# junejunejune/c_orb_slam

Measured on AMD Instinct MI355X. Metric: tracking FPS + ORB matches/sec, KITTI-00 stereo; local-BA iter/sec, higher is better.
Workload: dtype u8

## Files before the change

c_orb_slam_amd/csrc/octree.hip:

```cpp
#include "octree.hpp"

#include <cstdlib>

namespace orbgpu {

constexpr int OCT_TMAX = 1024;
constexpr int kOctCellsMax = kOctKMax / 2;

struct OctShared {
    int16_t x0[2 * kOctNMax], y0[2 * kOctNMax], x1[2 * kOctNMax], y1[2 * kOctNMax];
    uint16_t cnt[2 * kOctNMax], seq[2 * kOctNMax], kbeg[2 * kOctNMax];
    int16_t prv[2 * kOctNMax], nxt[2 * kOctNMax];
    int ia[4 * kOctNMax];
    uint16_t vpos[4 * kOctNMax];
    uint16_t er[kOctNMax], eidx[kOctNMax];
    uint16_t vs[kOctNMax], vs2[kOctNMax];
    uint32_t sk[kOctNMax];
    uint16_t knode[kOctKMax], arena[kOctKMax];
    alignas(16) uint16_t tmp[kOctKMax];
    int wsum[OCT_TMAX / 64];
    int head, size, nfree, m, newm, seqctr, flag;
};

template <int T, class Flag, class Put>
__device__ __forceinline__ int oct_scan(int n, Flag flag, Put put, int* wsum) {
    const int t = threadIdx.x, lane = t & 63, wid = t >> 6;
    const int per = (n + T - 1) / T;
    const int a = min(n, t * per), e = min(n, a + per);
    int local = 0;
    for (int i = a; i < e; i++) local += flag(i) ? 1 : 0;
    int incl = local;
#pragma unroll
    for (int o = 1; o < 64; o <<= 1) {
        const int y = __shfl_up(incl, o, 64);
        if (lane >= o) incl += y;
    }
    if (lane == 63) wsum[wid] = incl;
    __syncthreads();
    int off = 0, total = 0;
#pragma unroll
    for (int w = 0; w < T / 64; w++) {
        const int s = wsum[w];
        if (w < wid) off += s;
        total += s;
    }
    int ex = off + incl - local;
    for (int i = a; i < e; i++)
        if (flag(i)) put(i, ex++);
    __syncthreads();
    return total;
}

template <int T, class Val, class Put>
__device__ __forceinline__ int oct_scan_val(int n, Val val, Put put, int* wsum) {
    const int t = threadIdx.x, lane = t & 63, wid = t >> 6;
    const int per = (n + T - 1) / T;
    const int a = min(n, t * per), e = min(n, a + per);
    int local = 0;
    for (int i = a; i < e; i++) local += val(i);
    int incl = local;
#pragma unroll
    for (int o = 1; o < 64; o <<= 1) {
        const int y = __shfl_up(incl, o, 64);
        if (lane >= o) incl += y;
    }
    if (lane == 63) wsum[wid] = incl;
    __syncthreads();
    int off = 0, total = 0;
#pragma unroll
    for (int w = 0; w < T / 64; w++) {
        const int s = wsum[w];
        if (w < wid) off += s;
        total += s;
    }
    int ex = off + incl - local;
    for (int i = a; i < e; i++) {
        put(i, ex);
        ex += val(i);
    }
    __syncthreads();
    return total;
}

__device__ __forceinline__ void oct_child_rect(const OctShared& S, int p, int q, int& a0, int& b0, int& a1, int& b1) {
    const int X0 = S.x0[p], Y0 = S.y0[p], X1 = S.x1[p], Y1 = S.y1[p];
    const int halfX = (int)ceilf((float)(X1 - X0) / 2), halfY = (int)ceilf((float)(Y1 - Y0) / 2);
    const int mx = X0 + halfX, my = Y0 + halfY;
    a0 = (q & 1) ? mx : X0;
    a1 = (q & 1) ? X1 : mx;
    b0 = (q & 2) ? my : Y0;
    b1 = (q & 2) ? Y1 : my;
}

__device__ __forceinline__ int oct_quadrant(const OctShared& S, int p, uint32_t pk) {
    const int halfX = (int)ceilf((float)(S.x1[p] - S.x0[p]) / 2), halfY = (int)ceilf((float)(S.y1[p] - S.y0[p]) / 2);
    const int mx = S.x0[p] + halfX, my = S.y0[p] + halfY;
    const int x = (int)(pk & 0xfff), y = (int)((pk >> 12) & 0xfff);
    return (x < mx) ? (y < my ? 0 : 2) : (y < my ? 1 : 3);
}

__device__ __forceinline__ int oct_best_key(uint32_t pk, int k) { return (int)((pk >> 24) << 16) | (0xffff - k); }

template <int T>
__global__ void __launch_bounds__(T) k_octree(OctInput in, int nlevels, const OctLevelDev* __restrict__ lv,
                                                 uint32_t* __restrict__ jobsel, int* __restrict__ jobcnt, int jcap,
                                                 uint16_t* __restrict__ gscratch, size_t gstride, int* __restrict__ err) {
    __shared__ OctShared S;
    ORBGPU_PROF_START;
#ifdef ORBGPU_PROF
    struct JobTimer {
        unsigned long long t0;
        int lvl;
        __device__ ~JobTimer() {
            if (threadIdx.x == 0) {
                const unsigned long long c = clock64() - t0;
                atomicMax(&g_orbgpu_prof[10], (c << 4) | (unsigned long long)lvl);
                atomicAdd(&g_orbgpu_prof[11], c);
                atomicAdd(&g_orbgpu_prof[12], 1ull);
            }
        }
    } jt{(unsigned long long)clock64(), (int)blockIdx.x / ((int)gridDim.x / nlevels)};
#endif
    const int B = (int)gridDim.x / nlevels;
    const int l = (int)blockIdx.x / B, b = (int)blockIdx.x - l * B, job = b * nlevels + l;
    const int tid = threadIdx.x;
    const int cb = in.lcb[l], nc = in.lcb[l + 1] - cb;
    const int* cnt = in.counts + (size_t)b * in.ncells + cb;
    if (nc + 1 > 4 * kOctNMax || nc > kOctCellsMax) {
        if (tid == 0) {
            jobcnt[job] = 0;
            atomicOr(err, 2);
        }
        return;
    }
    int* cdelta = reinterpret_cast<int*>(S.tmp);
    const int n = oct_scan_val<T>(
        nc, [&](int i) { return cnt[i]; },
        [&](int i, int o) {
            S.ia[i] = o;
            cdelta[i] = in.cell_slot[cb + i] - in.cell_slot[cb] - o;
        },
        S.wsum);
    const size_t base = (size_t)b * in.slots_per_image + (size_t)in.cell_slot[cb];
    if (n <= 0 || n > 0xffff) {
        if (tid == 0) {
            jobcnt[job] = 0;
            if (n > 0xffff) atomicOr(err, 2);
        }
        return;
    }
    {
        const uint32_t* sl = in.slots + base;
        uint32_t* dst = in.packed + base;
        constexpr int U = 4;
        for (int k0 = tid; k0 < n; k0 += U * T) {
            uint32_t v[U];
#pragma unroll
            for (int u = 0; u < U; u++) {
                const int k = k0 + u * T;
                if (k < n) {
                    int lo = 0, hi = nc - 1;
                    while (lo < hi) {
                        const int mid = (lo + hi + 1) >> 1;
                        if (S.ia[mid] <= k) lo = mid;
                        else hi = mid - 1;
                    }
                    v[u] = sl[k + cdelta[lo]];
                }
            }
#pragma unroll
            for (int u = 0; u < U; u++)
                if (k0 + u * T < n) dst[k0 + u * T] = v[u];
        }
        if (tid == 0) atomicAdd(in.g_total, n);
    }
    __syncthreads();
    const uint32_t* src = in.packed + base;
    const OctLevelDev L = lv[l];
    const int N = L.N;
    uint16_t* knode = S.knode;
    uint16_t* arena = S.arena;
    uint16_t* tmp = S.tmp;
    if (n > kOctKMax) {
        knode = gscratch + base;
        arena = knode + gstride;
        tmp = arena + gstride;
    }
    const int W = L.maxX - L.minX, Hh = L.maxY - L.minY;
    const int nIni = (int)roundf((float)W / (float)Hh);
    if (nIni < 1 || nIni > kOctNMax) {
        if (tid == 0) {
            jobcnt[job] = 0;
            atomicOr(err, 4);
        }
        return;
    }
    const float hX = (float)W / (float)nIni;
    for (int i = tid; i < nIni; i += T) S.ia[i] = 0;
    __syncthreads();
    for (int k = tid; k < n; k += T) {
        const uint32_t pk = src[k];
        int ib = (int)((float)(pk & 0xfff) / hX);
        ib = min(ib, nIni - 1);
        knode[k] = (uint16_t)ib;
        atomicAdd(&S.ia[ib], 1);
    }
    __syncthreads();
    int cur = 0;
    int Sz = oct_scan<T>(
        nIni, [&](int i) { return S.ia[i] > 0; },
        [&](int i, int r) {
            S.x0[r] = (int16_t)(int)(hX * (float)i);
            S.x1[r] = (int16_t)(int)(hX * (float)(i + 1));
            S.y0[r] = 0;
            S.y1[r] = (int16_t)Hh;
            S.cnt[r] = (uint16_t)S.ia[i];
            S.seq[r] = (uint16_t)i;
            S.er[i] = (uint16_t)r;
        },
        S.wsum);
    for (int k = tid; k < n; k += T) knode[k] = S.er[knode[k]];
    int seqbase = nIni;
    int phase2 = 0, m = 0;
    __syncthreads();
    ORBGPU_PROF_MARK(0);
    for (;;) {
        const int prevSize = Sz;
        const int nE = oct_scan<T>(
            Sz, [&](int i) { return S.cnt[cur + i] > 1; },
            [&](int i, int r) {
                S.er[i] = (uint16_t)r;
                S.eidx[r] = (uint16_t)i;
            },
            S.wsum);
        ORBGPU_PROF_COUNT(9);
        if (nE == 0) break;
        for (int v = tid; v < 4 * nE; v += T) S.ia[v] = 0;
        __syncthreads();
        for (int k = tid; k < n; k += T) {
            const int p = knode[k];
            if (S.cnt[cur + p] > 1) {
                const int v = 4 * S.er[p] + oct_quadrant(S, cur + p, src[k]);
                tmp[k] = (uint16_t)v;
                atomicAdd(&S.ia[v], 1);
            } else {
                tmp[k] = 0xffff;
            }
        }
        __syncthreads();
        const int nC = oct_scan<T>(
            4 * nE, [&](int v) { return S.ia[v] > 0; }, [&](int v, int r) { S.vpos[v] = (uint16_t)r; }, S.wsum);
        const int nb = kOctNMax - cur;
        const int nNM = oct_scan<T>(
            Sz, [&](int i) { return S.cnt[cur + i] == 1; }, [&](int i, int r) { S.er[i] = (uint16_t)(nC + r); },
            S.wsum);
        if (nC + nNM > kOctNMax) {
            if (tid == 0) {
                jobcnt[job] = 0;
                atomicOr(err, 8);
            }
            return;
        }
        for (int v = tid; v < 4 * nE; v += T) {
            const int c = S.ia[v];
            if (c > 0) {
                const int t = S.vpos[v], pos = nC - 1 - t, parent = cur + S.eidx[v >> 2];
                int a0, b0, a1, b1;
                oct_child_rect(S, parent, v & 3, a0, b0, a1, b1);
                S.x0[nb + pos] = (int16_t)a0;
                S.y0[nb + pos] = (int16_t)b0;
                S.x1[nb + pos] = (int16_t)a1;
                S.y1[nb + pos] = (int16_t)b1;
                S.cnt[nb + pos] = (uint16_t)c;
                S.seq[nb + pos] = (uint16_t)(seqbase + t);
                S.vpos[v] = (uint16_t)pos;
            }
        }
        for (int i = tid; i < Sz; i += T)
            if (S.cnt[cur + i] == 1) {
                const int pos = S.er[i];
                S.x0[nb + pos] = S.x0[cur + i];
                S.y0[nb + pos] = S.y0[cur + i];
                S.x1[nb + pos] = S.x1[cur + i];
                S.y1[nb + pos] = S.y1[cur + i];
                S.cnt[nb + pos] = 1;
                S.seq[nb + pos] = S.seq[cur + i];
            }
        __syncthreads();
        const int nToExpand = oct_scan<T>(
            4 * nE, [&](int v) { return S.ia[v] > 1; }, [&](int v, int r) { S.vs[r] = (uint16_t)S.vpos[v]; },
            S.wsum);
        for (int k = tid; k < n; k += T) {
            const int v = tmp[k];
            knode[k] = v != 0xffff ? S.vpos[v] : S.er[knode[k]];
        }
        seqbase += nC;
        cur = nb;
        Sz = nC + nNM;
        __syncthreads();
        if (Sz >= N || Sz == prevSize) break;
        if (Sz + nToExpand * 3 > N) {
            phase2 = 1;
            m = nToExpand;
            break;
        }
    }
    ORBGPU_PROF_MARK(1);
    if (phase2) {
        const int nb = kOctNMax - cur;
        {
            oct_scan_val<T>(
                Sz, [&](int i) { return (int)S.cnt[cur + i]; }, [&](int i, int ex) { S.kbeg[cur + i] = (uint16_t)ex; },
                S.wsum);
            for (int i = tid; i < Sz; i += T) {
                S.ia[i] = 0;
                S.prv[cur + i] = (int16_t)(i > 0 ? cur + i - 1 : -1);
                S.nxt[cur + i] = (int16_t)(i + 1 < Sz ? cur + i + 1 : -1);
            }
            if (tid == 0) {
                S.head = Sz > 0 ? cur : -1;
                S.size = Sz;
                S.nfree = nb;
                S.seqctr = seqbase;
                S.m = m;
                S.flag = 0;
            }
            for (int i = tid; i < m; i += T) S.vs[i] = (uint16_t)(cur + S.vs[i]);
            __syncthreads();
            for (int k = tid; k < n; k += T) {
                const int p = knode[k];
                arena[S.kbeg[cur + p] + atomicAdd(&S.ia[p], 1)] = (uint16_t)k;
            }
            __syncthreads();
        }
        ORBGPU_PROF_MARK(2);
        for (;;) {
            ORBGPU_PROF_COUNT(8);
            const int prevSize = S.size;
            const int mm = S.m;
            for (int i = tid; i < mm; i += T) {
                const int id = S.vs[i];
                S.sk[i] = ((uint32_t)S.cnt[id] << 16) | S.seq[id];
            }
            __syncthreads();
            for (int i = tid; i < mm; i += T) {
                const uint32_t ki = S.sk[i];
                int r = 0;
                for (int j = 0; j < mm; j++) r += S.sk[j] < ki ? 1 : 0;
                S.vs2[r] = S.vs[i];
            }
            for (int i = tid; i < 4 * mm; i += T) S.ia[i] = 0;
            if (tid == 0) S.newm = 0;
            __syncthreads();
            ORBGPU_PROF_MARK(3);
            const int tot = oct_scan_val<T>(
                mm, [&](int j) { return (int)S.cnt[S.vs2[j]]; }, [&](int j, int ex) { S.er[j] = (uint16_t)ex; },
                S.wsum);
            auto owner = [&](int t) {
                int lo = 0, hi = mm - 1;
                while (lo < hi) {
                    const int mid = (lo + hi + 1) >> 1;
                    if ((int)S.er[mid] <= t) lo = mid;
                    else hi = mid - 1;
                }
                return lo;
            };
            for (int t = tid; t < tot; t += T) {
                const int j = owner(t), p = S.vs2[j], pos = S.kbeg[p] + (t - S.er[j]);
                const int k = arena[pos];
                const int q = oct_quadrant(S, p, src[k]);
                tmp[t] = (uint16_t)k;
                knode[t] = (uint16_t)(4 * j + q);
                atomicAdd(&S.ia[4 * j + q], 1);
            }
            __syncthreads();
            for (int j = tid; j < mm; j += T) {
                int start = S.kbeg[S.vs2[j]];
#pragma unroll
                for (int q = 0; q < 4; q++) {
                    S.vpos[4 * j + q] = (uint16_t)start;
                    start += S.ia[4 * j + q];
                    S.ia[4 * j + q] = 0;
                }
            }
            __syncthreads();
            for (int t = tid; t < tot; t += T) {
                const int v = knode[t];
                arena[S.vpos[v] + atomicAdd(&S.ia[v], 1)] = tmp[t];
            }
            __syncthreads();
            ORBGPU_PROF_MARK(4);
            if (tid == 0) {
                int head = S.head, size = S.size, nfree = S.nfree, seqctr = S.seqctr, newm = 0, flag = 0;
                for (int j = mm - 1; j >= 0; j--) {
                    const int p = S.vs2[j];
                    int c4[4];
#pragma unroll
                    for (int q = 0; q < 4; q++) c4[q] = S.ia[4 * j + q];
                    for (int q = 0; q < 4; q++) {
                        const int c = c4[q];
                        if (c > 0) {
                            const int id = nfree++;
                            if (nfree > 2 * kOctNMax || id == cur) {
                                flag = 1;
                                break;
                            }
                            int a0, b0, a1, b1;
                            oct_child_rect(S, p, q, a0, b0, a1, b1);
                            S.x0[id] = (int16_t)a0;
                            S.y0[id] = (int16_t)b0;
                            S.x1[id] = (int16_t)a1;
                            S.y1[id] = (int16_t)b1;
                            S.cnt[id] = (uint16_t)c;
                            S.seq[id] = (uint16_t)(seqctr++);
                            S.kbeg[id] = S.vpos[4 * j + q];
                            S.prv[id] = -1;
                            S.nxt[id] = (int16_t)head;
                            if (head >= 0) S.prv[head] = (int16_t)id;
                            head = id;
                            size++;
                            if (c > 1) S.vs[newm++] = (uint16_t)id;
                        }
                    }
                    if (flag) break;
                    const int pp = S.prv[p], pn = S.nxt[p];
                    if (pp >= 0) S.nxt[pp] = (int16_t)pn;
                    else head = pn;
                    if (pn >= 0) S.prv[pn] = (int16_t)pp;
                    S.prv[p] = -2;
                    size--;
                    if (size >= N) break;
                }
                S.head = head;
                S.size = size;
                S.nfree = nfree;
                S.seqctr = seqctr;
                S.newm = newm;
                S.flag = flag;
            }
            __syncthreads();
            ORBGPU_PROF_MARK(5);
            if (S.flag) {
                if (tid == 0) {
                    jobcnt[job] = 0;
                    atomicOr(err, 8);
                }
                return;
            }
            if (S.size >= N || S.size == prevSize) break;
            if (tid == 0) S.m = S.newm;
            __syncthreads();
        }
        const int n2 = S.nfree - nb;
        const int sz = oct_scan<T>(
            n2 + Sz,
            [&](int u) {
                const int id = u < n2 ? nb + n2 - 1 - u : cur + (u - n2);
                return S.prv[id] != -2;
            },
            [&](int u, int r) { S.vpos[r] = (uint16_t)(u < n2 ? nb + n2 - 1 - u : cur + (u - n2)); }, S.wsum);
        if (sz > jcap) {
            if (tid == 0) {
                jobcnt[job] = 0;
                atomicOr(err, 16);
            }
            return;
        }
        for (int i = tid; i < sz; i += T) {
            const int id = S.vpos[i];
            const int kb = S.kbeg[id], kc = S.cnt[id];
            for (int t = 0; t < kc; t++) tmp[kb + t] = (uint16_t)i;
            S.ia[i] = -1;
        }
        __syncthreads();
        for (int pos = tid; pos < n; pos += T) {
            const int k = arena[pos];
            atomicMax(&S.ia[tmp[pos]], oct_best_key(src[k], k));
        }
        __syncthreads();
        for (int i = tid; i < sz; i += T) {
            const int k = 0xffff - (S.ia[i] & 0xffff);
            jobsel[(size_t)job * jcap + i] = src[k];
        }
        if (tid == 0) jobcnt[job] = sz;
        ORBGPU_PROF_MARK(6);
        return;
    }
    if (Sz > jcap) {
        if (tid == 0) {
            jobcnt[job] = 0;
            atomicOr(err, 16);
        }
        return;
    }
    for (int i = tid; i < Sz; i += T) S.ia[i] = -1;
    __syncthreads();
    for (int k = tid; k < n; k += T) atomicMax(&S.ia[knode[k]], oct_best_key(src[k], k));
    __syncthreads();
    for (int i = tid; i < Sz; i += T) {
        const int k = 0xffff - (S.ia[i] & 0xffff);
        jobsel[(size_t)job * jcap + i] = src[k];
    }
    if (tid == 0) jobcnt[job] = Sz;
    ORBGPU_PROF_MARK(7);
}

__global__ void __launch_bounds__(64) k_sel_build(const uint32_t* __restrict__ jobsel, const int* __restrict__ jobcnt,
                                                  int nlevels, int jcap, int cap, int2* __restrict__ sel, int selcap,
                                                  int* __restrict__ nout, int* __restrict__ err) {
    const int b = blockIdx.x, lane = threadIdx.x;
    const int c = lane < nlevels ? jobcnt[b * nlevels + lane] : 0;
    int incl = c;
#pragma unroll
    for (int o = 1; o < 64; o <<= 1) {
        const int y = __shfl_up(incl, o, 64);
        if (lane >= o) incl += y;
    }
    const int total = __shfl(incl, 63, 64);
    if (lane == 0) {
        nout[b] = total;
        if (total > cap || total > selcap) atomicOr(err, 1);
    }
    if (total > cap || total > selcap) return;
    for (int l = 0; l < nlevels; l++) {
        const int cl = __shfl(c, l, 64), off = __shfl(incl - c, l, 64);
        const uint32_t* js = jobsel + (size_t)(b * nlevels + l) * jcap;
        for (int i = lane; i < cl; i += 64)
            sel[(size_t)b * selcap + off + i] = make_int2((int)js[i], (b << 20) | (l << 16) | (off + i));
    }
}

int octree_prof_read(unsigned long long* out16) {
#ifdef ORBGPU_PROF
    unsigned long long v[32];
    ORB_HIP_CHECK(hipMemcpyFromSymbol(v, HIP_SYMBOL(g_orbgpu_prof), sizeof(v)));
    for (int i = 0; i < 16; i++) out16[i] = v[i];
    unsigned long long z[32] = {};
    ORB_HIP_CHECK(hipMemcpyToSymbol(HIP_SYMBOL(g_orbgpu_prof), z, sizeof(z)));
    return 0;
#else
    (void)out16;
    return -1;
#endif
}

int octree_launch(const OctInput& in, int B, int nlevels, const OctLevelDev* lv, uint32_t* jobsel, int* jobcnt, int jcap,
                  uint16_t* gscratch, size_t gstride, int cap, int2* sel, int selcap, int* nout, int* err,
                  hipStream_t s) {
    static const int nt = [] {
        const char* e = getenv("ORBGPU_OCT_T");
        const int v = e ? atoi(e) : 512;
        return v == 256 || v == 1024 ? v : 512;
    }();
    if (nt == 1024)
        hipLaunchKernelGGL(k_octree<1024>, dim3(B * nlevels), dim3(1024), 0, s, in, nlevels, lv, jobsel, jobcnt,
                           jcap, gscratch, gstride, err);
    else if (nt == 512)
        hipLaunchKernelGGL(k_octree<512>, dim3(B * nlevels), dim3(512), 0, s, in, nlevels, lv, jobsel, jobcnt,
                           jcap, gscratch, gstride, err);
    else
        hipLaunchKernelGGL(k_octree<256>, dim3(B * nlevels), dim3(256), 0, s, in, nlevels, lv, jobsel, jobcnt,
                           jcap, gscratch, gstride, err);
    hipLaunchKernelGGL(k_sel_build, dim3(B), dim3(64), 0, s, (const uint32_t*)jobsel, (const int*)jobcnt, nlevels,
                       jcap, cap, sel, selcap, nout, err);
    ORB_HIP_CHECK(hipGetLastError());
    return 0;
}

}
```

c_orb_slam_amd/csrc/octree.hpp:

```cpp
#pragma once
#include <hip/hip_runtime.h>

#include <cstdint>

#include "orb_common.hpp"

namespace orbgpu {

constexpr int kOctNMax = 640;
constexpr int kOctKMax = 4096;

struct OctLevelDev {
    int minX, maxX, minY, maxY, N;
};

int octree_prof_read(unsigned long long* out16);

struct OctInput {
    const uint32_t* slots;
    size_t slots_per_image;
    const int* counts;
    const int* cell_slot;
    const int* lcb;
    int ncells;
    uint32_t* packed;
    int* g_total;
};

int octree_launch(const OctInput& in, int B, int nlevels, const OctLevelDev* lv, uint32_t* jobsel, int* jobcnt, int jcap,
                  uint16_t* gscratch, size_t gstride, int cap, int2* sel, int selcap, int* nout, int* err,
                  hipStream_t s);

}
```

c_orb_slam_amd/csrc/orb_extract.hip:

```cpp
#include "orb_extract.hpp"

#include <algorithm>
#include <atomic>
#include <chrono>
#include <cmath>
#include <cstring>
#include <thread>

namespace orbgpu {

__constant__ int8_t c_pattern[256 * 4];
__constant__ int8_t c_disc[2 * 1024];
__constant__ int c_ndisc;
__constant__ int c_umax[16];
__constant__ int c_gauss[7];

static const int8_t kPattern[256 * 4] = {
#include "brief_pattern.inc"
};

__device__ __forceinline__ int xcd_tile(int bid, int nb) { return (bid & 7) * (nb >> 3) + (bid >> 3); }
static inline unsigned grid8(int n) { return (unsigned)((n + 7) & ~7); }
constexpr int kFastSplitLevel = 3;

// ... 1444 lines not shown
    ORB_HIP_CHECK(hipMalloc(&d_blur_, blur_bytes_ * B));
    ORB_HIP_CHECK(hipMemset(d_blur_, 0, blur_bytes_ * B));
    ORB_HIP_CHECK(hipMalloc(&d_slots_, slots_per_image_ * 4 * B));
    ORB_HIP_CHECK(hipMalloc(&d_counts_, cells_.size() * 4 * B));
    ORB_HIP_CHECK(hipMalloc(&d_cells_, cells_.size() * sizeof(CellDesc)));
    ORB_HIP_CHECK(hipMemcpy(d_cells_, cells_.data(), cells_.size() * sizeof(CellDesc), hipMemcpyHostToDevice));
    ORB_HIP_CHECK(hipMalloc(&d_groups_, groups_.size() * sizeof(CellGroup)));
    ORB_HIP_CHECK(hipMemcpy(d_groups_, groups_.data(), groups_.size() * sizeof(CellGroup), hipMemcpyHostToDevice));
    ORB_HIP_CHECK(hipMalloc(&d_tiles_, tiles_.size() * sizeof(BlurTile)));
    ORB_HIP_CHECK(hipMemcpy(d_tiles_, tiles_.data(), tiles_.size() * sizeof(BlurTile), hipMemcpyHostToDevice));
    {
        std::vector<int> cs(cells_.size());
        for (size_t c = 0; c < cells_.size(); c++) cs[c] = cells_[c].slot_off;
        ORB_HIP_CHECK(hipMalloc(&d_cellslot_, std::max<size_t>(cs.size(), 1) * 4));
        ORB_HIP_CHECK(hipMemcpy(d_cellslot_, cs.data(), cs.size() * 4, hipMemcpyHostToDevice));
    }
    ORB_HIP_CHECK(hipMalloc(&d_lcb_, level_cell_begin_.size() * 4));
    ORB_HIP_CHECK(hipMemcpy(d_lcb_, level_cell_begin_.data(), level_cell_begin_.size() * 4, hipMemcpyHostToDevice));
    if (slots_per_image_ * B > ((size_t)1 << 30)) return -1;
    packed_cap_ = (int)(slots_per_image_ * B);
    ORB_HIP_CHECK(hipMalloc(&d_packed_, (size_t)packed_cap_ * 4));
    ORB_HIP_CHECK(hipMalloc(&d_hdr_, (size_t)B * (nlevels_ + 2) * 4 + 64));
    d_gtotal_ = (int*)((char*)d_hdr_ + (size_t)B * (nlevels_ + 2) * 4);
    d_gtotal_alias_ = true;
    sel_cap_ = B * std::max(nfeatures_ * 2 + 64, 256);
    ORB_HIP_CHECK(hipMalloc(&d_sel_, (size_t)sel_cap_ * sizeof(int2)));
    std::vector<LevelDev> ld(nlevels_);
    for (int l = 0; l < nlevels_; l++) {
        ld[l].off = levels_[l].off;
        ld[l].pitch = levels_[l].pitch;
        ld[l].scale = scale_[l];
        ld[l].boff = levels_[l].boff;
        ld[l].bpitch = levels_[l].bpitch;
        ld[l].kp_size = (float)(int)(kPatch * scale_[l]);
    }
    if (nlevels_ > kMaxLevels) return -1;
    for (int l = 0; l < nlevels_; l++) levelArgs_.lv[l] = ld[l];
    ORB_HIP_CHECK(hipMalloc(&d_levels_, ld.size() * sizeof(LevelDev)));
    ORB_HIP_CHECK(hipMemcpy(d_levels_, ld.data(), ld.size() * sizeof(LevelDev), hipMemcpyHostToDevice));
    ORB_HIP_CHECK(hipMalloc(&d_tabs_, std::max<size_t>(tabs.size(), 16)));
    if (!tabs.empty()) ORB_HIP_CHECK(hipMemcpy(d_tabs_, tabs.data(), tabs.size(), hipMemcpyHostToDevice));
    F(d_jobsel_); F(d_jobcnt_); F(d_octlv_); F(d_gscr_); F(d_nout_);
    jcap_ = 0;
    std::vector<OctLevelDev> ol(nlevels_);
    for (int l = 0; l < nlevels_; l++) {
        ol[l].minX = kEdge - 3;
        ol[l].maxX = levels_[l].w - kEdge + 3;
        ol[l].minY = kEdge - 3;
        ol[l].maxY = levels_[l].h - kEdge + 3;
        ol[l].N = nPerLevel_[l];
        jcap_ = std::max(jcap_, nPerLevel_[l] + 8);
    }
    if (jcap_ > kOctNMax) return -1;
    selcap_ = jcap_ * nlevels_;
    ORB_HIP_CHECK(hipMalloc(&d_octlv_, ol.size() * sizeof(OctLevelDev)));
    ORB_HIP_CHECK(hipMemcpy(d_octlv_, ol.data(), ol.size() * sizeof(OctLevelDev), hipMemcpyHostToDevice));
    ORB_HIP_CHECK(hipMalloc(&d_jobsel_, (size_t)B * nlevels_ * jcap_ * 4));
    ORB_HIP_CHECK(hipMalloc(&d_jobcnt_, (size_t)B * nlevels_ * 4));
    ORB_HIP_CHECK(hipMalloc(&d_gscr_, (size_t)packed_cap_ * 3 * 2));
    ORB_HIP_CHECK(hipMalloc(&d_nout_, (size_t)(B + 1) * 4));
    ORB_HIP_CHECK(hipFree(d_sel_));
    d_sel_ = nullptr;
    sel_cap_ = selcap_ * B;
    ORB_HIP_CHECK(hipMalloc(&d_sel_, (size_t)sel_cap_ * sizeof(int2)));
    if (h_nout_) (void)hipHostFree(h_nout_);
    ORB_HIP_CHECK(hipHostMalloc((void**)&h_nout_, (size_t)(B + 1) * 4));
    geomW_ = W;
    geomH_ = H;
    return 0;
}

int Extractor::extract(const uint8_t* imgs, int B, int W, int H, int step, size_t img_stride,
                       bool imgs_on_device, orb_kp* kps, uint8_t* desc, int cap, bool out_on_device,
                       int* n_out, const uint8_t* const* list) {
    if (B <= 0 || B > maxB_ || W <= 0 || H <= 0) return -1;
    if (W > maxW_ || H > maxH_) return -1;
    if (int e = setup_geometry(W, H)) return e;
    hipStream_t s = stream_;
    const uint8_t* src = imgs;
    if (!imgs_on_device) {
        const size_t need = img_stride * (B - 1) + (size_t)step * (H - 1) + W;
        if (need > in_cap_) {
            if (d_in_) (void)hipFree(d_in_);
            ORB_HIP_CHECK(hipMalloc(&d_in_, need));
            in_cap_ = need;
        }
        if (h_in_) ORB_HIP_CHECK(hipEventSynchronize(ev_[0]));
        if (need > h_in_cap_) {
            if (h_in_) (void)hipHostFree(h_in_);
            h_in_ = nullptr;
            h_in_cap_ = 0;
            ORB_HIP_CHECK(hipHostMalloc(&h_in_, need));
            h_in_cap_ = need;
        }
        if (list) {
            const size_t one = (size_t)step * (H - 1) + W;
            for (int b = 0; b < B; b++) std::memcpy((uint8_t*)h_in_ + img_stride * b, list[b], one);
        } else {
            std::memcpy(h_in_, imgs, need);
        }
        ORB_HIP_CHECK(hipMemcpyAsync(d_in_, h_in_, need, hipMemcpyHostToDevice, s));
        src = (const uint8_t*)d_in_;
    }
    ORB_HIP_CHECK(hipEventRecord(ev_[0], s));
    const int ncells = (int)cells_.size();
    if (work_B_ != B && build_work(B)) return -2;
    const bool split = fastSplit_ && work_part_[0] > 0 && work_part_[1] > 0;
    int planFlags = (split ? kPlanFastSplit : 0) | (evBlur_ ? kPlanBlurSide : 0) | (B >= 8 ? kPlanTile32 : 0);
    int planChainFrom = 0;
    {
        const LevelHost& L0 = levels_[0];
        const int n = (L0.pitch / 16) * L0.ph;
// ... 31 lines not shown
            const LevelHost& P = levels_[l - 1];
            const uint8_t* T = (const uint8_t*)d_tabs_;
            const int v = B >= 8 ? 1 : 0, pb = v * (nlevels_ + 1) + l;
            const int nt = ptile_n_[v * nlevels_ + l];
            auto kern = v ? k_pyr_resize<kPyrTileH[1]> : k_pyr_resize<kPyrTileH[0]>;
            hipLaunchKernelGGL(kern, dim3(grid8(nt), B), dim3(256), plds_[v * nlevels_ + l], s, (uint8_t*)d_pyr_, img_bytes_,
                               P.off, P.pitch, L.off, L.pitch, L.ph, L.w, L.h,
                               (const int*)(T + tab_off_[l][0]), (const short2*)(T + tab_off_[l][1]),
                               (const int2*)(T + tab_off_[l][2]), (const short2*)(T + tab_off_[l][3]),
                               (const PyrTile*)d_ptiles_ + ptile_begin_[pb], nt);
        }
        if (!flow && lend < nlevels_) {
            const uint8_t* T = (const uint8_t*)d_chain_;
            const LevelHost& P = levels_[lend - 1];
            hipLaunchKernelGGL(k_pyr_chain, dim3(chainK_, B), dim3(256), chainLds_, s, (uint8_t*)d_pyr_, img_bytes_,
                               (long long)P.off, P.pitch, P.w, (const ChainLevel*)T, nlevels_ - lend,
                               (const int4*)(T + chainStripOff_), (const uint16_t*)(T + chainRowOff_),
                               (const uint8_t*)d_tabs_, chainSrcLds_, chainSrcRp_);
        }
    }
    ORB_HIP_CHECK(hipGetLastError());
    ORB_HIP_CHECK(hipEventRecord(ev_[1], s));
    static const bool blurEarly = [] {
        const char* e = getenv("ORBGPU_BLUR_EARLY");
        return e && e[0] == '1';
    }();
    if (blurEarly && !evBlur_) {
        planFlags |= kPlanBlurEarly;
        hipLaunchKernelGGL(k_blur7, dim3(grid8((int)tiles_.size()), B), dim3(256), 0, s, (const uint8_t*)d_pyr_,
                           (uint8_t*)d_blur_, img_bytes_, blur_bytes_, (const BlurTile*)d_tiles_, (int)tiles_.size());
    }
    if (evBlur_) {
        ORB_HIP_CHECK(hipStreamWaitEvent(side_, ev_[1], 0));
        hipLaunchKernelGGL(k_blur7, dim3(grid8((int)tiles_.size()), B), dim3(256), 0, side_, (const uint8_t*)d_pyr_,
                           (uint8_t*)d_blur_, img_bytes_, blur_bytes_, (const BlurTile*)d_tiles_, (int)tiles_.size());
        ORB_HIP_CHECK(hipEventRecord(evBlur_, side_));
    }
    if (split) {
        hipLaunchKernelGGL(k_fast_cells, dim3(work_part_[1]), dim3(256), 0, s, (const uint8_t*)d_pyr_, img_bytes_,
                           (const CellGroup*)d_groups_, iniTh_, minTh_, (uint32_t*)d_slots_, slots_per_image_,
                           (int*)d_counts_, ncells, (const int*)d_work_ + work_part_[0]);
        ORB_HIP_CHECK(hipStreamWaitEvent(s, evFastA_, 0));
    } else {
        hipLaunchKernelGGL(k_fast_cells, dim3(work_n_), dim3(256), 0, s, (const uint8_t*)d_pyr_, img_bytes_,
                           (const CellGroup*)d_groups_, iniTh_, minTh_, (uint32_t*)d_slots_, slots_per_image_,
                           (int*)d_counts_, ncells, (const int*)d_work_);
    }
    ORB_HIP_CHECK(hipGetLastError());
    ORB_HIP_CHECK(hipEventRecord(ev_[3], s));
    ORB_HIP_CHECK(hipEventRecord(ev_[4], s));
    int* d_err = (int*)d_nout_ + B;
    OctInput oin{(const uint32_t*)d_slots_, slots_per_image_, (const int*)d_counts_, (const int*)d_cellslot_,
                 (const int*)d_lcb_, ncells, (uint32_t*)d_packed_, d_gtotal_};
    if (int e = octree_launch(oin, B, nlevels_, (const OctLevelDev*)d_octlv_, (uint32_t*)d_jobsel_, (int*)d_jobcnt_,
                              jcap_, (uint16_t*)d_gscr_, (size_t)packed_cap_, cap, (int2*)d_sel_, selcap_,
                              (int*)d_nout_, d_err, s))
        return e;
    ORB_HIP_CHECK(hipEventRecord(ev_[5], s));
    if (evBlur_)
        ORB_HIP_CHECK(hipStreamWaitEvent(s, evBlur_, 0));
    else if (!blurEarly)
        hipLaunchKernelGGL(k_blur7, dim3(grid8((int)tiles_.size()), B), dim3(256), 0, s, (const uint8_t*)d_pyr_,
                           (uint8_t*)d_blur_, img_bytes_, blur_bytes_, (const BlurTile*)d_tiles_, (int)tiles_.size());
    ORB_HIP_CHECK(hipEventRecord(ev_[2], s));
    orb_kp_dev* okps = (orb_kp_dev*)kps;
    uint8_t* odesc = desc;
    if (!out_on_device) {
        const size_t nk = (size_t)B * cap;
        if (nk > out_cap_) {
            if (d_kps_) (void)hipFree(d_kps_);
            if (d_desc_) (void)hipFree(d_desc_);
            ORB_HIP_CHECK(hipMalloc(&d_kps_, nk * sizeof(orb_kp_dev)));
            ORB_HIP_CHECK(hipMalloc(&d_desc_, nk * 32));
            out_cap_ = nk;
        }
        okps = (orb_kp_dev*)d_kps_;
        odesc = (uint8_t*)d_desc_;
    }
    {
        const int gx = (selcap_ + 3) / 4;
        const int nwg = B >= 8 ? gx * 8 * ((B + 7) / 8) : gx * B;
        hipLaunchKernelGGL(k_orient_desc, dim3(nwg), dim3(256), 0, s, (const uint8_t*)d_pyr_,
                           (const uint8_t*)d_blur_, img_bytes_, blur_bytes_, (const int2*)d_sel_, selcap_,
                           (const int*)d_nout_, levelArgs_, okps, odesc, cap, gx, B);
    }
    ORB_HIP_CHECK(hipGetLastError());
    ORB_HIP_CHECK(hipMemcpyAsync(h_nout_, d_nout_, (size_t)(B + 1) * 4, hipMemcpyDeviceToHost, s));
    ORB_HIP_CHECK(hipEventRecord(ev_[6], s));
    ORB_HIP_CHECK(stream_wait(s));
    const int err = h_nout_[B];
    for (int b = 0; b < B; b++) n_out[b] = h_nout_[b];
    if (err & 1) return -3;
    if (err) return -1;
    if (!out_on_device) {
        for (int b = 0; b < B; b++) {
            if (n_out[b] == 0) continue;
            ORB_HIP_CHECK(hipMemcpyAsync(kps + (size_t)b * cap, okps + (size_t)b * cap, (size_t)n_out[b] * sizeof(orb_kp_dev),
                                         hipMemcpyDeviceToHost, s));
            ORB_HIP_CHECK(hipMemcpyAsync(desc + (size_t)b * cap * 32, odesc + (size_t)b * cap * 32, (size_t)n_out[b] * 32,
                                         hipMemcpyDeviceToHost, s));
        }
        ORB_HIP_CHECK(stream_wait(s));
    }
    last_B_ = B;
    planFlags_ = planFlags;
    planChainFrom_ = planChainFrom;
    return 0;
}

// ... 66 lines not shown
```

c_orb_slam_amd/csrc/orb_extract.hpp:

```cpp
#pragma once
#include <atomic>
#include <condition_variable>
#include <cstddef>
#include <cstdint>
#include <mutex>
#include <thread>
#include <vector>
#include <array>

#include "orb_common.hpp"
#include "octree.hpp"
#include "../../include/orbslam_gpu.h"

namespace orbgpu {

struct orb_kp_dev {
    float x, y, size, angle, response;
    int32_t octave, class_id;
};
static_assert(sizeof(orb_kp_dev) == 28, "cv::KeyPoint layout");

struct CellDesc {
    int r0, r1, c0, c1;
    int offx, offy;
// ... 104 lines not shown
    int maxW_ = 0, maxH_ = 0, maxB_ = 0;
    int geomW_ = -1, geomH_ = -1;
    std::vector<LevelHost> levels_;
    LevelArgs levelArgs_{};
    std::vector<CellDesc> cells_;
    std::vector<CellGroup> groups_;
    std::vector<int> level_cell_begin_;
    std::vector<BlurTile> tiles_;
    std::vector<PyrTile> ptiles_;
    std::vector<int> ptile_begin_, ptile_n_, plds_;
    std::vector<int> ptile_th_;
    bool flow_ = false;
    int* d_flowcnt_ = nullptr;
    int flowBands_[2] = {0, 0}, flowLds_[2] = {0, 0};
    FlowArgs flow_args(int v, int B) const;
    int plan_chain(const std::vector<std::vector<int>>& yr);
    bool chain_ = false;
    int chainK_ = 0, chainLds_ = 0, chainFrom_ = 0, chainSrcLds_ = 0, chainSrcRp_ = 0;
    std::vector<std::vector<int>> xofsAll_;
    std::vector<std::vector<short>> xalAll_;
    size_t chainStripOff_ = 0, chainRowOff_ = 0;
    std::vector<uint8_t> chainTab_;
    void* d_chain_ = nullptr;
    void* d_cellslot_ = nullptr;
    std::vector<std::array<size_t, 4>> tab_off_;
    size_t img_bytes_ = 0, blur_bytes_ = 0, slots_per_image_ = 0;
    int packed_cap_ = 0, sel_cap_ = 0;
    int last_B_ = 0;
    int planFlags_ = 0, planChainFrom_ = 0;

    hipStream_t stream_ = nullptr;
    bool ownStream_ = true;
    int lent_ = 0;
    hipEvent_t ev_[7] = {};
    hipStream_t side_ = nullptr;
    hipEvent_t evBlur_ = nullptr;
    bool fastSplit_ = false;
    hipEvent_t evPyrA_ = nullptr, evFastA_ = nullptr;
    void *d_in_ = nullptr, *d_pyr_ = nullptr, *d_blur_ = nullptr, *d_slots_ = nullptr, *d_counts_ = nullptr;
    void *d_ptiles_ = nullptr;
    void *d_cells_ = nullptr, *d_tiles_ = nullptr, *d_lcb_ = nullptr, *d_packed_ = nullptr, *d_hdr_ = nullptr;
    void *d_sel_ = nullptr, *d_levels_ = nullptr, *d_tabs_ = nullptr, *d_kps_ = nullptr, *d_desc_ = nullptr;
    int* d_gtotal_ = nullptr;
    void* d_work_ = nullptr;
    void* d_groups_ = nullptr;
    int work_B_ = -1, work_n_ = 0;
    int work_part_[2] = {0, 0};
    bool d_gtotal_alias_ = false;
    size_t in_cap_ = 0, out_cap_ = 0;
    void* h_in_ = nullptr;
    size_t h_in_cap_ = 0;
    void *d_jobsel_ = nullptr, *d_jobcnt_ = nullptr, *d_octlv_ = nullptr, *d_gscr_ = nullptr, *d_nout_ = nullptr;
    int jcap_ = 0, selcap_ = 0;
    int* h_nout_ = nullptr;

};

int debug_prof_extract(unsigned long long* out32);

}
```

Before: 44000.

## Restructure octree distribution to drop keypoint arena and shrink shared memory

The octree kernel now templates its shared node storage on a node capacity. A small variant is picked on the host when every level's needs fit, which cuts LDS footprint and may raise occupancy. Keys are kept in LDS when they fit. The per-keypoint arena, kbeg and tmp bucketing is replaced by recomputing quadrants from each key's node id, and two scans are merged into one packed 16-bit dual-count scan. This removes the scatter passes and their scratch memory, at the cost of rescanning all keypoints on every phase-2 iteration and heavier lambda-based branching between LDS and global paths.

After: 43720. About the same (-0.6%).

```diff
diff --git a/c_orb_slam_amd/csrc/octree.hip b/c_orb_slam_amd/csrc/octree.hip
--- a/c_orb_slam_amd/csrc/octree.hip
+++ b/c_orb_slam_amd/csrc/octree.hip
@@ -1,5 +1,7 @@
 #include "octree.hpp"
 
+#include <cmath>
+#include <cstddef>
 #include <cstdlib>
 
 namespace orbgpu {
@@ -7,20 +9,26 @@
 constexpr int OCT_TMAX = 1024;
 constexpr int kOctCellsMax = kOctKMax / 2;
 
+template <int NC>
 struct OctShared {
-    int16_t x0[2 * kOctNMax], y0[2 * kOctNMax], x1[2 * kOctNMax], y1[2 * kOctNMax];
-    uint16_t cnt[2 * kOctNMax], seq[2 * kOctNMax], kbeg[2 * kOctNMax];
-    int16_t prv[2 * kOctNMax], nxt[2 * kOctNMax];
-    int ia[4 * kOctNMax];
-    uint16_t vpos[4 * kOctNMax];
-    uint16_t er[kOctNMax], eidx[kOctNMax];
-    uint16_t vs[kOctNMax], vs2[kOctNMax];
-    uint32_t sk[kOctNMax];
-    uint16_t knode[kOctKMax], arena[kOctKMax];
-    alignas(16) uint16_t tmp[kOctKMax];
+    static constexpr int NN = NC + kOctNMax;
+    int16_t x0[NN], y0[NN], x1[NN], y1[NN];
+    uint16_t cnt[NN], seq[NN];
+    uint16_t jof[NN];
+    int16_t prv[NN], nxt[NN];
+    int ia[4 * NC];
+    uint16_t vpos[4 * NC];
+    uint16_t er[NC], eidx[NC];
+    uint16_t vs[NC], vs2[NC];
+    alignas(16) uint32_t sk[NC + 4];
+    alignas(16) uint16_t knode[kOctKMax];
+    uint32_t keys[kOctKMax];
     int wsum[OCT_TMAX / 64];
-    int head, size, nfree, m, newm, seqctr, flag;
+    int head, size, nfree, m, newm, seqctr, flag, jdone;
 };
+static_assert(offsetof(OctShared<kOctNSmall>, seq) >= kOctCellsMax * sizeof(int), "cell deltas over x0..cnt");
+static_assert(kOctKMax * sizeof(uint16_t) >= kOctCellsMax * sizeof(int), "cell offsets over knode");
+static_assert(kOctNSmall <= kOctNMax && 4 * kOctNMax < 0x10000, "packed 16-bit scan counters");
 
 template <int T, class Flag, class Put>
 __device__ __forceinline__ int oct_scan(int n, Flag flag, Put put, int* wsum) {
@@ -82,7 +90,8 @@
     return total;
 }
 
-__device__ __forceinline__ void oct_child_rect(const OctShared& S, int p, int q, int& a0, int& b0, int& a1, int& b1) {
+template <class Sh>
+__device__ __forceinline__ void oct_child_rect(const Sh& S, int p, int q, int& a0, int& b0, int& a1, int& b1) {
     const int X0 = S.x0[p], Y0 = S.y0[p], X1 = S.x1[p], Y1 = S.y1[p];
     const int halfX = (int)ceilf((float)(X1 - X0) / 2), halfY = (int)ceilf((float)(Y1 - Y0) / 2);
     const int mx = X0 + halfX, my = Y0 + halfY;
@@ -92,7 +101,8 @@
     b1 = (q & 2) ? Y1 : my;
 }
 
-__device__ __forceinline__ int oct_quadrant(const OctShared& S, int p, uint32_t pk) {
+template <class Sh>
+__device__ __forceinline__ int oct_quadrant(const Sh& S, int p, uint32_t pk) {
     const int halfX = (int)ceilf((float)(S.x1[p] - S.x0[p]) / 2), halfY = (int)ceilf((float)(S.y1[p] - S.y0[p]) / 2);
     const int mx = S.x0[p] + halfX, my = S.y0[p] + halfY;
     const int x = (int)(pk & 0xfff), y = (int)((pk >> 12) & 0xfff);
@@ -101,11 +111,11 @@
 
 __device__ __forceinline__ int oct_best_key(uint32_t pk, int k) { return (int)((pk >> 24) << 16) | (0xffff - k); }
 
-template <int T>
+template <int T, int NC>
 __global__ void __launch_bounds__(T) k_octree(OctInput in, int nlevels, const OctLevelDev* __restrict__ lv,
                                                  uint32_t* __restrict__ jobsel, int* __restrict__ jobcnt, int jcap,
-                                                 uint16_t* __restrict__ gscratch, size_t gstride, int* __restrict__ err) {
-    __shared__ OctShared S;
+                                                 uint16_t* __restrict__ gscratch, int* __restrict__ err) {
+    __shared__ OctShared<NC> S;
     ORBGPU_PROF_START;
 #ifdef ORBGPU_PROF
     struct JobTimer {
@@ -126,18 +136,19 @@
     const int tid = threadIdx.x;
     const int cb = in.lcb[l], nc = in.lcb[l + 1] - cb;
     const int* cnt = in.counts + (size_t)b * in.ncells + cb;
-    if (nc + 1 > 4 * kOctNMax || nc > kOctCellsMax) {
+    if (nc > kOctCellsMax) {
         if (tid == 0) {
             jobcnt[job] = 0;
             atomicOr(err, 2);
         }
         return;
     }
-    int* cdelta = reinterpret_cast<int*>(S.tmp);
+    int* coff = reinterpret_cast<int*>(S.knode);
+    int* cdelta = reinterpret_cast<int*>(S.x0);
     const int n = oct_scan_val<T>(
         nc, [&](int i) { return cnt[i]; },
         [&](int i, int o) {
-            S.ia[i] = o;
+            coff[i] = o;
             cdelta[i] = in.cell_slot[cb + i] - in.cell_slot[cb] - o;
         },
         S.wsum);
@@ -149,6 +160,7 @@
         }
         return;
     }
+    const bool lds = n <= kOctKMax;
     {
         const uint32_t* sl = in.slots + base;
         uint32_t* dst = in.packed + base;
@@ -162,7 +174,7 @@
                     int lo = 0, hi = nc - 1;
                     while (lo < hi) {
                         const int mid = (lo + hi + 1) >> 1;
-                        if (S.ia[mid] <= k) lo = mid;
+                        if (coff[mid] <= k) lo = mid;
                         else hi = mid - 1;
                     }
                     v[u] = sl[k + cdelta[lo]];
@@ -170,25 +182,27 @@
             }
 #pragma unroll
             for (int u = 0; u < U; u++)
-                if (k0 + u * T < n) dst[k0 + u * T] = v[u];
+                if (k0 + u * T < n) {
+                    if (lds) S.keys[k0 + u * T] = v[u];
+                    else dst[k0 + u * T] = v[u];
+                }
         }
         if (tid == 0) atomicAdd(in.g_total, n);
     }
     __syncthreads();
     const uint32_t* src = in.packed + base;
+    uint16_t* gnode = gscratch + base;
+    auto key = [&](int k) -> uint32_t { return lds ? S.keys[k] : src[k]; };
+    auto node_of = [&](int k) -> int { return lds ? (int)S.knode[k] : (int)gnode[k]; };
+    auto set_node = [&](int k, int v) {
+        if (lds) S.knode[k] = (uint16_t)v;
+        else gnode[k] = (uint16_t)v;
+    };
     const OctLevelDev L = lv[l];
     const int N = L.N;
-    uint16_t* knode = S.knode;
-    uint16_t* arena = S.arena;
-    uint16_t* tmp = S.tmp;
-    if (n > kOctKMax) {
-        knode = gscratch + base;
-        arena = knode + gstride;
-        tmp = arena + gstride;
-    }
     const int W = L.maxX - L.minX, Hh = L.maxY - L.minY;
     const int nIni = (int)roundf((float)W / (float)Hh);
-    if (nIni < 1 || nIni > kOctNMax) {
+    if (nIni < 1 || nIni > NC) {
         if (tid == 0) {
             jobcnt[job] = 0;
             atomicOr(err, 4);
@@ -199,10 +213,10 @@
     for (int i = tid; i < nIni; i += T) S.ia[i] = 0;
     __syncthreads();
     for (int k = tid; k < n; k += T) {
-        const uint32_t pk = src[k];
+        const uint32_t pk = key(k);
         int ib = (int)((float)(pk & 0xfff) / hX);
         ib = min(ib, nIni - 1);
-        knode[k] = (uint16_t)ib;
+        set_node(k, ib);
         atomicAdd(&S.ia[ib], 1);
     }
     __syncthreads();
@@ -219,42 +233,48 @@
             S.er[i] = (uint16_t)r;
         },
         S.wsum);
-    for (int k = tid; k < n; k += T) knode[k] = S.er[knode[k]];
+    for (int k = tid; k < n; k += T) set_node(k, S.er[node_of(k)]);
     int seqbase = nIni;
-    int phase2 = 0, m = 0;
+    int phase2 = 0, m = 0, lastC = 0;
     __syncthreads();
     ORBGPU_PROF_MARK(0);
     for (;;) {
         const int prevSize = Sz;
-        const int nE = oct_scan<T>(
-            Sz, [&](int i) { return S.cnt[cur + i] > 1; },
+        for (int v = tid; v < 4 * Sz; v += T) S.ia[v] = 0;
+        const int nE = oct_scan_val<T>(
+            Sz, [&](int i) { return S.cnt[cur + i] > 1 ? 1 : 0; },
             [&](int i, int r) {
-                S.er[i] = (uint16_t)r;
-                S.eidx[r] = (uint16_t)i;
+                if (S.cnt[cur + i] > 1) {
+                    S.er[i] = (uint16_t)r;
+                    S.eidx[r] = (uint16_t)i;
+                } else {
+                    S.er[i] = (uint16_t)(i - r);
+                }
             },
             S.wsum);
         ORBGPU_PROF_COUNT(9);
         if (nE == 0) break;
-        for (int v = tid; v < 4 * nE; v += T) S.ia[v] = 0;
+        for (int k = tid; k < n; k += T) {
+            const int p = node_of(k);
+            if (S.cnt[cur + p] > 1) atomicAdd(&S.ia[4 * S.er[p] + oct_quadrant(S, cur + p, key(k))], 1);
+        }
         __syncthreads();
-        for (int k = tid; k < n; k += T) {
-            const int p = knode[k];
-            if (S.cnt[cur + p] > 1) {
-                const int v = 4 * S.er[p] + oct_quadrant(S, cur + p, src[k]);
-                tmp[k] = (uint16_t)v;
-                atomicAdd(&S.ia[v], 1);
-            } else {
-                tmp[k] = 0xffff;
-            }
-        }
-        __syncthreads();
-        const int nC = oct_scan<T>(
-            4 * nE, [&](int v) { return S.ia[v] > 0; }, [&](int v, int r) { S.vpos[v] = (uint16_t)r; }, S.wsum);
-        const int nb = kOctNMax - cur;
-        const int nNM = oct_scan<T>(
-            Sz, [&](int i) { return S.cnt[cur + i] == 1; }, [&](int i, int r) { S.er[i] = (uint16_t)(nC + r); },
+        const int tot = oct_scan_val<T>(
+            4 * nE,
+            [&](int v) {
+                const int c = S.ia[v];
+                return (c > 0 ? 1 : 0) | (c > 1 ? 0x10000 : 0);
+            },
+            [&](int v, int r) {
+                const int c = S.ia[v];
+                if (c > 0) S.vpos[v] = (uint16_t)(r & 0xffff);
+                if (c > 1 && (r >> 16) < NC) S.vs[r >> 16] = (uint16_t)(r & 0xffff);
+            },
             S.wsum);
-        if (nC + nNM > kOctNMax) {
+        const int nC = tot & 0xffff, nToExpand = tot >> 16;
+        const int nNM = Sz - nE;
+        const int nb = NC - cur;
+        if (nC + nNM > NC) {
             if (tid == 0) {
                 jobcnt[job] = 0;
                 atomicOr(err, 8);
@@ -273,12 +293,11 @@
                 S.y1[nb + pos] = (int16_t)b1;
                 S.cnt[nb + pos] = (uint16_t)c;
                 S.seq[nb + pos] = (uint16_t)(seqbase + t);
-                S.vpos[v] = (uint16_t)pos;
             }
         }
         for (int i = tid; i < Sz; i += T)
             if (S.cnt[cur + i] == 1) {
-                const int pos = S.er[i];
+                const int pos = nC + S.er[i];
                 S.x0[nb + pos] = S.x0[cur + i];
                 S.y0[nb + pos] = S.y0[cur + i];
                 S.x1[nb + pos] = S.x1[cur + i];
@@ -286,15 +305,15 @@
                 S.cnt[nb + pos] = 1;
                 S.seq[nb + pos] = S.seq[cur + i];
             }
-        __syncthreads();
-        const int nToExpand = oct_scan<T>(
-            4 * nE, [&](int v) { return S.ia[v] > 1; }, [&](int v, int r) { S.vs[r] = (uint16_t)S.vpos[v]; },
-            S.wsum);
         for (int k = tid; k < n; k += T) {
-            const int v = tmp[k];
-            knode[k] = v != 0xffff ? S.vpos[v] : S.er[knode[k]];
+            const int p = node_of(k);
+            if (S.cnt[cur + p] > 1)
+                set_node(k, nC - 1 - S.vpos[4 * S.er[p] + oct_quadrant(S, cur + p, key(k))]);
+            else
+                set_node(k, nC + S.er[p]);
         }
         seqbase += nC;
+        lastC = nC;
         cur = nb;
         Sz = nC + nNM;
         __syncthreads();
@@ -307,30 +326,24 @@
     }
     ORBGPU_PROF_MARK(1);
     if (phase2) {
-        const int nb = kOctNMax - cur;
+        auto pid = [&](int a) { return a < cur ? a : a + NC; };
         {
-            oct_scan_val<T>(
-                Sz, [&](int i) { return (int)S.cnt[cur + i]; }, [&](int i, int ex) { S.kbeg[cur + i] = (uint16_t)ex; },
-                S.wsum);
             for (int i = tid; i < Sz; i += T) {
-                S.ia[i] = 0;
                 S.prv[cur + i] = (int16_t)(i > 0 ? cur + i - 1 : -1);
                 S.nxt[cur + i] = (int16_t)(i + 1 < Sz ? cur + i + 1 : -1);
             }
+            for (int i = tid; i < OctShared<NC>::NN; i += T) S.jof[i] = 0xffff;
+            if (cur)
+                for (int k = tid; k < n; k += T) set_node(k, cur + node_of(k));
             if (tid == 0) {
                 S.head = Sz > 0 ? cur : -1;
                 S.size = Sz;
-                S.nfree = nb;
+                S.nfree = 0;
                 S.seqctr = seqbase;
                 S.m = m;
                 S.flag = 0;
             }
-            for (int i = tid; i < m; i += T) S.vs[i] = (uint16_t)(cur + S.vs[i]);
-            __syncthreads();
-            for (int k = tid; k < n; k += T) {
-                const int p = knode[k];
-                arena[S.kbeg[cur + p] + atomicAdd(&S.ia[p], 1)] = (uint16_t)k;
-            }
+            for (int i = tid; i < m; i += T) S.vs[i] = (uint16_t)(cur + lastC - 1 - S.vs[i]);
             __syncthreads();
         }
         ORBGPU_PROF_MARK(2);
@@ -342,56 +355,31 @@
                 const int id = S.vs[i];
                 S.sk[i] = ((uint32_t)S.cnt[id] << 16) | S.seq[id];
             }
+            if (tid < 4) S.sk[mm + tid] = 0xffffffffu;
             __syncthreads();
             for (int i = tid; i < mm; i += T) {
                 const uint32_t ki = S.sk[i];
+                const uint4* s4 = reinterpret_cast<const uint4*>(S.sk);
                 int r = 0;
-                for (int j = 0; j < mm; j++) r += S.sk[j] < ki ? 1 : 0;
-                S.vs2[r] = S.vs[i];
+                for (int j = 0; j < (mm + 3) >> 2; j++) {
+                    const uint4 v = s4[j];
+                    r += (v.x < ki ? 1 : 0) + (v.y < ki ? 1 : 0) + (v.z < ki ? 1 : 0) + (v.w < ki ? 1 : 0);
+                }
+                const int id = S.vs[i];
+                S.vs2[r] = (uint16_t)id;
+                S.jof[id] = (uint16_t)r;
             }
             for (int i = tid; i < 4 * mm; i += T) S.ia[i] = 0;
-            if (tid == 0) S.newm = 0;
             __syncthreads();
             ORBGPU_PROF_MARK(3);
-            const int tot = oct_scan_val<T>(
-                mm, [&](int j) { return (int)S.cnt[S.vs2[j]]; }, [&](int j, int ex) { S.er[j] = (uint16_t)ex; },
-                S.wsum);
-            auto owner = [&](int t) {
-                int lo = 0, hi = mm - 1;
-                while (lo < hi) {
-                    const int mid = (lo + hi + 1) >> 1;
-                    if ((int)S.er[mid] <= t) lo = mid;
-                    else hi = mid - 1;
-                }
-                return lo;
-            };
-            for (int t = tid; t < tot; t += T) {
-                const int j = owner(t), p = S.vs2[j], pos = S.kbeg[p] + (t - S.er[j]);
-                const int k = arena[pos];
-                const int q = oct_quadrant(S, p, src[k]);
-                tmp[t] = (uint16_t)k;
-                knode[t] = (uint16_t)(4 * j + q);
-                atomicAdd(&S.ia[4 * j + q], 1);
-            }
-            __syncthreads();
-            for (int j = tid; j < mm; j += T) {
-                int start = S.kbeg[S.vs2[j]];
-#pragma unroll
-                for (int q = 0; q < 4; q++) {
-                    S.vpos[4 * j + q] = (uint16_t)start;
-                    start += S.ia[4 * j + q];
-                    S.ia[4 * j + q] = 0;
-                }
-            }
-            __syncthreads();
-            for (int t = tid; t < tot; t += T) {
-                const int v = knode[t];
-                arena[S.vpos[v] + atomicAdd(&S.ia[v], 1)] = tmp[t];
+            for (int k = tid; k < n; k += T) {
+                const int p = node_of(k), j = S.jof[p];
+                if (j != 0xffff) atomicAdd(&S.ia[4 * j + oct_quadrant(S, p, key(k))], 1);
             }
             __syncthreads();
             ORBGPU_PROF_MARK(4);
             if (tid == 0) {
-                int head = S.head, size = S.size, nfree = S.nfree, seqctr = S.seqctr, newm = 0, flag = 0;
+                int head = S.head, size = S.size, nfree = S.nfree, seqctr = S.seqctr, newm = 0, flag = 0, jdone = mm;
                 for (int j = mm - 1; j >= 0; j--) {
                     const int p = S.vs2[j];
                     int c4[4];
@@ -400,11 +388,11 @@
                     for (int q = 0; q < 4; q++) {
                         const int c = c4[q];
                         if (c > 0) {
-                            const int id = nfree++;
-                            if (nfree > 2 * kOctNMax || id == cur) {
+                            if (nfree >= kOctNMax) {
                                 flag = 1;
                                 break;
                             }
+                            const int id = pid(nfree++);
                             int a0, b0, a1, b1;
                             oct_child_rect(S, p, q, a0, b0, a1, b1);
                             S.x0[id] = (int16_t)a0;
@@ -413,7 +401,7 @@
                             S.y1[id] = (int16_t)b1;
                             S.cnt[id] = (uint16_t)c;
                             S.seq[id] = (uint16_t)(seqctr++);
-                            S.kbeg[id] = S.vpos[4 * j + q];
+                            S.vpos[4 * j + q] = (uint16_t)id;
                             S.prv[id] = -1;
                             S.nxt[id] = (int16_t)head;
                             if (head >= 0) S.prv[head] = (int16_t)id;
@@ -429,6 +417,7 @@
                     if (pn >= 0) S.prv[pn] = (int16_t)pp;
                     S.prv[p] = -2;
                     size--;
+                    jdone = j;
                     if (size >= N) break;
                 }
                 S.head = head;
@@ -437,6 +426,7 @@
                 S.seqctr = seqctr;
                 S.newm = newm;
                 S.flag = flag;
+                S.jdone = jdone;
             }
             __syncthreads();
             ORBGPU_PROF_MARK(5);
@@ -447,18 +437,23 @@
                 }
                 return;
             }
+            const int jdone = S.jdone;
+            for (int k = tid; k < n; k += T) {
+                const int p = node_of(k), j = S.jof[p];
+                if (j != 0xffff && j >= jdone) set_node(k, S.vpos[4 * j + oct_quadrant(S, p, key(k))]);
+            }
             if (S.size >= N || S.size == prevSize) break;
             if (tid == 0) S.m = S.newm;
             __syncthreads();
         }
-        const int n2 = S.nfree - nb;
+        const int n2 = S.nfree;
         const int sz = oct_scan<T>(
             n2 + Sz,
             [&](int u) {
-                const int id = u < n2 ? nb + n2 - 1 - u : cur + (u - n2);
+                const int id = u < n2 ? pid(n2 - 1 - u) : cur + (u - n2);
                 return S.prv[id] != -2;
             },
-            [&](int u, int r) { S.vpos[r] = (uint16_t)(u < n2 ? nb + n2 - 1 - u : cur + (u - n2)); }, S.wsum);
+            [&](int u, int r) { S.jof[u < n2 ? pid(n2 - 1 - u) : cur + (u - n2)] = (uint16_t)r; }, S.wsum);
         if (sz > jcap) {
             if (tid == 0) {
                 jobcnt[job] = 0;
@@ -466,21 +461,13 @@
             }
             return;
         }
-        for (int i = tid; i < sz; i += T) {
-            const int id = S.vpos[i];
-            const int kb = S.kbeg[id], kc = S.cnt[id];
-            for (int t = 0; t < kc; t++) tmp[kb + t] = (uint16_t)i;
-            S.ia[i] = -1;
-        }
+        for (int i = tid; i < sz; i += T) S.ia[i] = -1;
         __syncthreads();
-        for (int pos = tid; pos < n; pos += T) {
-            const int k = arena[pos];
-            atomicMax(&S.ia[tmp[pos]], oct_best_key(src[k], k));
-        }
+        for (int k = tid; k < n; k += T) atomicMax(&S.ia[S.jof[node_of(k)]], oct_best_key(key(k), k));
         __syncthreads();
         for (int i = tid; i < sz; i += T) {
             const int k = 0xffff - (S.ia[i] & 0xffff);
-            jobsel[(size_t)job * jcap + i] = src[k];
+            jobsel[(size_t)job * jcap + i] = key(k);
         }
         if (tid == 0) jobcnt[job] = sz;
         ORBGPU_PROF_MARK(6);
@@ -495,11 +482,11 @@
     }
     for (int i = tid; i < Sz; i += T) S.ia[i] = -1;
     __syncthreads();
-    for (int k = tid; k < n; k += T) atomicMax(&S.ia[knode[k]], oct_best_key(src[k], k));
+    for (int k = tid; k < n; k += T) atomicMax(&S.ia[node_of(k)], oct_best_key(key(k), k));
     __syncthreads();
     for (int i = tid; i < Sz; i += T) {
         const int k = 0xffff - (S.ia[i] & 0xffff);
-        jobsel[(size_t)job * jcap + i] = src[k];
+        jobsel[(size_t)job * jcap + i] = key(k);
     }
     if (tid == 0) jobcnt[job] = Sz;
     ORBGPU_PROF_MARK(7);
@@ -544,23 +531,37 @@
 #endif
 }
 
-int octree_launch(const OctInput& in, int B, int nlevels, const OctLevelDev* lv, uint32_t* jobsel, int* jobcnt, int jcap,
-                  uint16_t* gscratch, size_t gstride, int cap, int2* sel, int selcap, int* nout, int* err,
+int octree_node_capacity(const OctLevelDev* lv, int nlevels) {
+    int need = 0;
+    for (int l = 0; l < nlevels; l++) {
+        const float r = roundf((float)(lv[l].maxX - lv[l].minX) / (float)(lv[l].maxY - lv[l].minY));
+        if (!(r >= 0.f && r <= (float)kOctNMax)) return kOctNMax;
+        need = std::max(need, std::max(lv[l].N + 8, 4 * (int)r));
+    }
+    return need <= kOctNSmall ? kOctNSmall : kOctNMax;
+}
+
+template <int T, int NC>
+static void octree_launch_as(const OctInput& in, int B, int nlevels, const OctLevelDev* lv, uint32_t* jobsel,
+                             int* jobcnt, int jcap, uint16_t* gscratch, int* err, hipStream_t s) {
+    hipLaunchKernelGGL((k_octree<T, NC>), dim3(B * nlevels), dim3(T), 0, s, in, nlevels, lv, jobsel, jobcnt, jcap,
+                       gscratch, err);
+}
+
+int octree_launch(const OctInput& in, int B, int nlevels, const OctLevelDev* lv, int node_cap, uint32_t* jobsel,
+                  int* jobcnt, int jcap, uint16_t* gscratch, int cap, int2* sel, int selcap, int* nout, int* err,
                   hipStream_t s) {
     static const int nt = [] {
         const char* e = getenv("ORBGPU_OCT_T");
         const int v = e ? atoi(e) : 512;
         return v == 256 || v == 1024 ? v : 512;
     }();
-    if (nt == 1024)
-        hipLaunchKernelGGL(k_octree<1024>, dim3(B * nlevels), dim3(1024), 0, s, in, nlevels, lv, jobsel, jobcnt,
-                           jcap, gscratch, gstride, err);
-    else if (nt == 512)
-        hipLaunchKernelGGL(k_octree<512>, dim3(B * nlevels), dim3(512), 0, s, in, nlevels, lv, jobsel, jobcnt,
-                           jcap, gscratch, gstride, err);
-    else
-        hipLaunchKernelGGL(k_octree<256>, dim3(B * nlevels), dim3(256), 0, s, in, nlevels, lv, jobsel, jobcnt,
-                           jcap, gscratch, gstride, err);
+    if (node_cap != kOctNSmall && node_cap != kOctNMax) return -1;
+    const bool small = node_cap == kOctNSmall;
+    auto go = nt == 1024 ? (small ? octree_launch_as<1024, kOctNSmall> : octree_launch_as<1024, kOctNMax>)
+              : nt == 512 ? (small ? octree_launch_as<512, kOctNSmall> : octree_launch_as<512, kOctNMax>)
+                          : (small ? octree_launch_as<256, kOctNSmall> : octree_launch_as<256, kOctNMax>);
+    go(in, B, nlevels, lv, jobsel, jobcnt, jcap, gscratch, err, s);
     hipLaunchKernelGGL(k_sel_build, dim3(B), dim3(64), 0, s, (const uint32_t*)jobsel, (const int*)jobcnt, nlevels,
                        jcap, cap, sel, selcap, nout, err);
     ORB_HIP_CHECK(hipGetLastError());
diff --git a/c_orb_slam_amd/csrc/octree.hpp b/c_orb_slam_amd/csrc/octree.hpp
--- a/c_orb_slam_amd/csrc/octree.hpp
+++ b/c_orb_slam_amd/csrc/octree.hpp
@@ -8,6 +8,7 @@
 namespace orbgpu {
 
 constexpr int kOctNMax = 640;
+constexpr int kOctNSmall = 320;
 constexpr int kOctKMax = 4096;
 
 struct OctLevelDev {
@@ -27,8 +28,10 @@
     int* g_total;
 };
 
-int octree_launch(const OctInput& in, int B, int nlevels, const OctLevelDev* lv, uint32_t* jobsel, int* jobcnt, int jcap,
-                  uint16_t* gscratch, size_t gstride, int cap, int2* sel, int selcap, int* nout, int* err,
+int octree_node_capacity(const OctLevelDev* lv, int nlevels);
+
+int octree_launch(const OctInput& in, int B, int nlevels, const OctLevelDev* lv, int node_cap, uint32_t* jobsel,
+                  int* jobcnt, int jcap, uint16_t* gscratch, int cap, int2* sel, int selcap, int* nout, int* err,
                   hipStream_t s);
 
 }
diff --git a/c_orb_slam_amd/csrc/orb_extract.hip b/c_orb_slam_amd/csrc/orb_extract.hip
--- a/c_orb_slam_amd/csrc/orb_extract.hip
+++ b/c_orb_slam_amd/csrc/orb_extract.hip
@@ -1520,12 +1520,13 @@
         jcap_ = std::max(jcap_, nPerLevel_[l] + 8);
     }
     if (jcap_ > kOctNMax) return -1;
+    octNodeCap_ = octree_node_capacity(ol.data(), nlevels_);
     selcap_ = jcap_ * nlevels_;
     ORB_HIP_CHECK(hipMalloc(&d_octlv_, ol.size() * sizeof(OctLevelDev)));
     ORB_HIP_CHECK(hipMemcpy(d_octlv_, ol.data(), ol.size() * sizeof(OctLevelDev), hipMemcpyHostToDevice));
     ORB_HIP_CHECK(hipMalloc(&d_jobsel_, (size_t)B * nlevels_ * jcap_ * 4));
     ORB_HIP_CHECK(hipMalloc(&d_jobcnt_, (size_t)B * nlevels_ * 4));
-    ORB_HIP_CHECK(hipMalloc(&d_gscr_, (size_t)packed_cap_ * 3 * 2));
+    ORB_HIP_CHECK(hipMalloc(&d_gscr_, (size_t)packed_cap_ * 2));
     ORB_HIP_CHECK(hipMalloc(&d_nout_, (size_t)(B + 1) * 4));
     ORB_HIP_CHECK(hipFree(d_sel_));
     d_sel_ = nullptr;
@@ -1663,9 +1664,9 @@
     int* d_err = (int*)d_nout_ + B;
     OctInput oin{(const uint32_t*)d_slots_, slots_per_image_, (const int*)d_counts_, (const int*)d_cellslot_,
                  (const int*)d_lcb_, ncells, (uint32_t*)d_packed_, d_gtotal_};
-    if (int e = octree_launch(oin, B, nlevels_, (const OctLevelDev*)d_octlv_, (uint32_t*)d_jobsel_, (int*)d_jobcnt_,
-                              jcap_, (uint16_t*)d_gscr_, (size_t)packed_cap_, cap, (int2*)d_sel_, selcap_,
-                              (int*)d_nout_, d_err, s))
+    if (int e = octree_launch(oin, B, nlevels_, (const OctLevelDev*)d_octlv_, octNodeCap_, (uint32_t*)d_jobsel_,
+                              (int*)d_jobcnt_, jcap_, (uint16_t*)d_gscr_, cap, (int2*)d_sel_, selcap_, (int*)d_nout_,
+                              d_err, s))
         return e;
     ORB_HIP_CHECK(hipEventRecord(ev_[5], s));
     if (evBlur_)
diff --git a/c_orb_slam_amd/csrc/orb_extract.hpp b/c_orb_slam_amd/csrc/orb_extract.hpp
--- a/c_orb_slam_amd/csrc/orb_extract.hpp
+++ b/c_orb_slam_amd/csrc/orb_extract.hpp
@@ -180,6 +180,7 @@
     size_t h_in_cap_ = 0;
     void *d_jobsel_ = nullptr, *d_jobcnt_ = nullptr, *d_octlv_ = nullptr, *d_gscr_ = nullptr, *d_nout_ = nullptr;
     int jcap_ = 0, selcap_ = 0;
+    int octNodeCap_ = 0;
     int* h_nout_ = nullptr;
 
 };
```
